# bastienjacquet/CudaDepthMapIntegration

Measured on AMD Instinct MI355X. Metric: Gvoxel-projections/s, higher is better.
Workload: dtype f64

## Files before the change

### cudadepthmapintegration_amd/csrc/dmi_capi_fuse.hip

```cpp
#include "dmi_context.h"

#include <algorithm>
#include <cmath>
#include <cstdlib>
#include <cstring>

using dmi::drain_events;
using dmi::EventPair;
using dmi::fail;
using dmi::flush_zero_fill;
using dmi::FuseArgs;
using dmi::FuseConfig;
using dmi::guarded;
using dmi::MapRec;
using dmi::TileArgs;
using dmi::TileMapRec;

namespace {

int sync_maps(dmi_context *ctx) {
  dmi_context::Views &v = ctx->views;
  const size_t n = v.h_maps.size();
  const size_t cap = std::max<size_t>(64, n * 2);
  bool fresh = false;
// ... 121 lines not shown
  unsigned long long mingled = 0, without = 0, strips = 0, pixels = 0;
  for (const dmi::Batch &bt : v.batches) {
    mingled += bt.mingled_strips;
    without += bt.holes;
    strips += (unsigned long long)bt.n * (unsigned long long)v.W * (unsigned long long)(v.H / 8);
    pixels += (unsigned long long)bt.n * (unsigned long long)v.W * (unsigned long long)v.H;
  }
  return dmi::hole_traits(mingled, without, strips, pixels);
}

int tile_geometry(dmi_context *ctx, const FuseArgs &a, const FuseConfig &cfg, const dmi::TileShape &sh, bool whole_grid, TileArgs *out) {
  TileArgs &t = *out;
  t.nx = a.nx; t.ny = a.ny; t.nz = a.nz; t.W = a.W; t.H = a.H;
  t.first_map = a.first_map; t.n_maps = a.n_maps; t.init_from_grid = a.init_from_grid;
  t.kpad = (a.nz + sh.tk - 1) / sh.tk * sh.tk;
  t.bricks_x = (a.nx + 8 * sh.wx - 1) / (8 * sh.wx);
  t.bricks_y = (a.ny + 8 * sh.wy - 1) / (8 * sh.wy);
  t.bricks_z = t.kpad / sh.tk;
  t.super_x = (t.bricks_x + 3) / 4;
  t.super_y = (t.bricks_y + 3) / 4;
  t.super_z = (t.bricks_z + 1) / 2;
  if (!whole_grid) {
    t.sbz_first = a.k_first / (2 * sh.tk);
    t.super_z = (a.k_first + a.k_count + 2 * sh.tk - 1) / (2 * sh.tk) - t.sbz_first;
  }
  if (t.bricks_x > 2047 || t.bricks_y > 2047 || t.bricks_z > 1023)
    return fail(ctx, DMI_ERR_INVALID_ARGUMENT, "dmi_fuse: more bricks along an axis than the tiled kernel's order entries hold");
  t.slot_base = t.sbz_first * t.super_x * t.super_y * 32;
  t.slot_count = t.super_x * t.super_y * t.super_z * 32;
  const int rc = slot_permutation(ctx, t.super_x, t.super_y, t.super_z, (cfg.variant & dmi::VAR_ZMAJOR_SLOTS) != 0, &t.sb_perm);
  if (rc != DMI_OK) return rc;
  t.xcd_run_wg = 32 * std::max(1, t.super_x * t.super_y);
  if (((int64_t)t.super_x * t.super_y * t.super_z * 32 + 16 * (int64_t)t.xcd_run_wg + 64) > (int64_t)0x7fffffff)
    return fail(ctx, DMI_ERR_INVALID_ARGUMENT, "dmi_fuse: grid too large for one launch");
  t.depth_bytes = (int32_t)((int64_t)a.W * a.H * (ctx->views.depth_f64 ? 8 : 4));
  t.kz0 = a.kz0;
  t.ox = a.ox; t.oy = a.oy; t.oz = a.oz; t.sx = a.sx; t.sy = a.sy; t.sz = a.sz;
  std::memcpy(t.g, a.g, sizeof(t.g));
  t.thick = a.thick; t.delta = a.delta; t.rho_pos = a.rho_pos; t.rho_neg = a.rho_neg;
  t.slope = a.slope; t.free_space = a.free_space;
  t.tile_maps = ctx->views.tile_maps.as<TileMapRec>();
  t.grid = a.grid; t.voxel_hits = a.voxel_hits; t.map_hits = a.map_hits;
  t.rotated = dmi::grid_axis_aligned(ctx->grid) ? 0 : 1;
  t.flags = ((cfg.variant & dmi::VAR_NO_INTERIOR) ? dmi::TILE_FLAG_NO_INTERIOR : 0) |
            ((cfg.variant & dmi::VAR_XCD_RUNS) ? dmi::TILE_FLAG_XCD_RUNS : 0);
  t.maps = ctx->views.maps.as<MapRec>();
  t.wbricks_x = (a.nx + 7) / 8;
  t.wbricks_y = (a.ny + 7) / 8;
  return DMI_OK;
}

int cz_table(dmi_context *ctx, const FuseArgs &a, TileArgs *t) {
  const size_t table_doubles = std::max<size_t>(ctx->views.h_maps.size(), 4) * (size_t)t->kpad;
  const size_t need = table_doubles + (size_t)dmi::kFreeSumsMax + 1;
  const int rc = dmi::ensure_idle_buffer(ctx, ctx->tables.cz_table, need * 8, need * 2 * 8);
  if (rc != DMI_OK) return rc;
  t->cz_table = ctx->tables.cz_table.as<double>();
  if (!a.init_from_grid && !ctx->opt.count_hits && a.n_maps <= dmi::kFreeSumsMax) t->free_sums = t->cz_table + table_doubles;
  return DMI_OK;
}

int zero_row(dmi_context *ctx, TileArgs *t) {
  bool fresh = false;
  const int rc = dmi::ensure_idle_buffer(ctx, ctx->tables.zero_row, (uint64_t)t->class_pitch, (uint64_t)t->class_pitch, &fresh);
  if (rc != DMI_OK) return rc;
  if (fresh) DMI_HIP(ctx, hipMemsetAsync(ctx->tables.zero_row.ptr, dmi::BRICK_MIXED, (size_t)t->class_pitch, ctx->stream));
  t->classes = ctx->tables.zero_row.as<uint8_t>();
  t->class_pitch = 0;
  return DMI_OK;
}

int class_table(dmi_context *ctx, const dmi::TileShape &sh, bool windows, TileArgs *t) {
  const size_t fine_bytes = ((size_t)t->wbricks_x * t->wbricks_y * t->bricks_z * (size_t)t->class_pitch + 255) / 256 * 256;
  const size_t coarse_end = (fine_bytes + (size_t)dmi::coarse_class_bytes(*t, sh.tk) + 255) / 256 * 256;
  const size_t cbytes = coarse_end + (windows ? fine_bytes * sizeof(dmi::WinPair) : 0);
  ctx->tables.coarse_offset = fine_bytes;
  bool fresh = false;
  const int rc = dmi::ensure_idle_buffer(ctx, ctx->tables.classes, cbytes, cbytes, &fresh);
  if (rc != DMI_OK) return rc;
  if (fresh) DMI_HIP(ctx, hipMemsetAsync(ctx->tables.classes.ptr, dmi::BRICK_SKIP, cbytes, ctx->stream));
  t->classes = ctx->tables.classes.as<uint8_t>();
  if (windows) {
    t->win_origin = reinterpret_cast<dmi::WinPair *>(ctx->tables.classes.as<uint8_t>() + coarse_end);
    t->win_delta = (int64_t)reinterpret_cast<intptr_t>(t->win_origin) - 16 * (int64_t)reinterpret_cast<intptr_t>(t->classes);
    t->win_recs = ctx->views.win_recs.as<dmi::WinRec>();
    t->foot_recs = ctx->views.foot_recs.as<dmi::FootRec>();
    t->vb_bytes = (int32_t)std::min<int64_t>(dmi::valid_bits_bytes(ctx->views.W, ctx->views.H), 0x7fffffff);
    t->vb_rowskip = (dmi::valid_bits_tiles_x(ctx->views.W) - 1) * 128;
    t->win_cx = dmi::kValidMargin + ctx->views.W / 2;
    t->win_cy = dmi::kValidMargin + ctx->views.H / 2;
  }
  return DMI_OK;
}

int order_tables(dmi_context *ctx, const dmi::TileShape &sh, int variant, TileArgs *t) {
  const size_t n_slots = (size_t)t->super_x * t->super_y * t->super_z * 32;
  const size_t order_bytes = (n_slots + 1) * sizeof(int32_t), level_bytes = dmi::order_scratch_bytes(n_slots);
  const int rc = dmi::ensure_idle_buffers(ctx, {{&ctx->tables.order, order_bytes, order_bytes}, {&ctx->tables.order_level, level_bytes, level_bytes}});
  if (rc != DMI_OK) return rc;
  t->order = ctx->tables.order.as<int32_t>() + 1;
  t->n_order = ctx->tables.order.as<int32_t>();
  t->order_levels = reinterpret_cast<const int32_t *>(ctx->tables.order_level.as<uint8_t>() + (n_slots + 15) / 16 * 16);
  t->xcd_run_wg = 32 * (4 / (sh.wx * sh.wy));
  if (dmi::cost_order(sh.wx * sh.wy, variant, n_slots)) {
    t->flags |= dmi::TILE_FLAG_COST_ORDER | dmi::TILE_FLAG_XCD_RUNS;
    t->xcd_run_wg = 16;
  }
  return DMI_OK;
}

#ifdef DMI_TUNING
int tuning_hooks(dmi_context *ctx, TileArgs *out) {
  TileArgs &t = *out;
  if (std::getenv("DMI_DEBUG_NO_DEPTH_LOADS")) t.depth_bytes = 0;
  if (std::getenv("DMI_DEBUG_WG_TIMES")) {
    const size_t per_round = 8 * (size_t)t.xcd_run_wg;
    const size_t blocks = ((size_t)t.super_x * t.super_y * t.super_z * 32 + 32 + per_round - 1) / per_round * per_round;
    const size_t bytes = (blocks * 3 + 2) * sizeof(unsigned long long);
    const int rc = dmi::ensure_idle_buffer(ctx, ctx->tables.wg_times, bytes, bytes);
    if (rc != DMI_OK) return rc;
    ctx->tables.wg_times_blocks = blocks;
    DMI_HIP(ctx, hipMemsetAsync(ctx->tables.wg_times.ptr, 0, bytes, ctx->stream));
    t.wg_times = ctx->tables.wg_times.as<unsigned long long>();
    t.wg_times_n = (int64_t)blocks;
  }
  if (const char *e = std::getenv("DMI_DEBUG_PAIRS")) {
    if (!std::strcmp(e, "nowin")) t.flags |= dmi::TILE_FLAG_DBG_SKIP_WINDOW_PAIRS;
    if (!std::strcmp(e, "onlywin")) t.flags |= dmi::TILE_FLAG_DBG_ONLY_WINDOW_PAIRS;
    if (!std::strcmp(e, "nowinloads")) t.flags |= dmi::TILE_FLAG_DBG_NO_WINDOW_LOADS;
  }
  if (const char *e = std::getenv("DMI_XCD_RUN_WG")) {
    t.xcd_run_wg = std::max(1, std::atoi(e));
    if (((int64_t)t.super_x * t.super_y * t.super_z * 32 + 8 * (int64_t)t.xcd_run_wg) > (int64_t)0x7fffffff)
      return fail(ctx, DMI_ERR_INVALID_ARGUMENT, "dmi_fuse: DMI_XCD_RUN_WG makes the launch too large");
  }
  return DMI_OK;
}
#endif

int tile_tables(dmi_context *ctx, const FuseArgs &a, FuseConfig *cfg, const dmi::TileShape &sh, const dmi::HoleTraits &traits, TileArgs *out) {
  TileArgs &t = *out;
  int rc = cz_table(ctx, a, &t);
  if (rc == DMI_OK) rc = dmi::ensure_buffer(ctx, ctx->tables.queue_heads, 128 * sizeof(int32_t));
  if (rc != DMI_OK) return rc;
  t.queue_heads = ctx->tables.queue_heads.as<int32_t>();
  if (dmi::fuse_without_classes(cfg->variant, (int64_t)t.wbricks_x * t.wbricks_y * (int64_t)t.bricks_z, a.n_maps))
    cfg->variant |= dmi::VAR_NO_BRICK_CLASSES;
  t.class_pitch = dmi::class_table_pitch((int32_t)ctx->views.h_maps.size());
  const bool zero_free = dmi::zero_free(a.init_from_grid != 0, ctx->volume.grid_free_of_negative_zero, ctx->opt.count_hits != 0, cfg->variant);
  if (cfg->variant & dmi::VAR_NO_BRICK_CLASSES) {
    rc = zero_row(ctx, &t);
  } else {
    bool any_tier1 = false;
    for (int32_t m = a.first_map; m < a.first_map + a.n_maps && !any_tier1; ++m) any_tier1 = std::isfinite(ctx->views.h_win_recs[(size_t)m].e_abs);
    dmi::WindowsQuestion q;
    q.tier1 = DMI_TIER1 != 0;
    q.general_k = cfg->general_k != 0;
    q.count_hits = cfg->count_hits != 0;
    q.variant = cfg->variant;
    q.holes = cfg->holes != 0;
    q.many_borders = traits.many_borders;
    q.any_tier1 = any_tier1;
    q.zero_free = zero_free;
    q.depth_f64 = ctx->views.depth_f64;
    rc = class_table(ctx, sh, dmi::use_windows(q), &t);
    if (rc == DMI_OK && !(cfg->variant & dmi::VAR_SPATIAL_ORDER)) rc = order_tables(ctx, sh, cfg->variant, &t);
  }
// ... 200 lines not shown
```

### cudadepthmapintegration_amd/csrc/fusion_classify.hip

```cpp
#include <algorithm>
#include <cstring>

#include <stdlib.h>

#include "fusion_kernels.h"
#include "fusion_device.h"

namespace dmi {

namespace {

template <typename T>
__device__ __forceinline__ T cload(const T *p) {
  return *reinterpret_cast<const T __attribute__((address_space(4))) *>(reinterpret_cast<uintptr_t>(p));
}

__device__ __forceinline__ float float_below(double d) {
  float f = (float)d;
  if ((double)f > d) f = nextafterf(f, -__builtin_inff());
  return f;
}
__device__ __forceinline__ float float_above(double d) {
  float f = (float)d;
  if ((double)f < d) f = nextafterf(f, __builtin_inff());
// ... 474 lines not shown
    TileMapRec tr_u;
    if constexpr (views_per_wave == 1) {
      const int mu = __builtin_amdgcn_readfirstlane(m);
      const MapRec *src = maps + mu;
      const TileMapRec *tsrc = a.tile_maps + mu;
#pragma unroll
      for (int q = 8; q < 12; ++q) mr_u.rt[q] = cload(&src->rt[q]);
      mr_u.pyramid = cload(&src->pyramid);
      tr_u.px = cload(&tsrc->px); tr_u.py = cload(&tsrc->py); tr_u.pz = cload(&tsrc->pz); tr_u.p0 = cload(&tsrc->p0);
      tr_u.qx = cload(&tsrc->qx); tr_u.qy = cload(&tsrc->qy); tr_u.qz = cload(&tsrc->qz); tr_u.q0 = cload(&tsrc->q0);
      tr_u.err = cload(&tsrc->err);
      tr_u.cz_err = cload(&tsrc->cz_err);
      tr_u.errz = cload(&tsrc->errz);
      if constexpr (GK) {
        tr_u.sx = cload(&tsrc->sx); tr_u.sy = cload(&tsrc->sy); tr_u.sz = cload(&tsrc->sz); tr_u.s0 = cload(&tsrc->s0);
      }
      mr = &mr_u;
      if (mine) {
        fp = box_footprint<ROT, GK>(a, &mr_u, &tr_u, bx * 8, bx * 8 + 7, by * 8, by * 8 + 7, bz * tk, bz * tk + tk - 1);
      }
    } else {
      if (mine) fp = box_footprint<ROT, GK>(a, mr, a.tile_maps + m, bx * 8, bx * 8 + 7, by * 8, by * 8 + 7, bz * tk, bz * tk + tk - 1);
    }
    const bool query = mine && (fp.query || fp.partial);
    uint8_t cls = fp.cls;
    const int li = query ? query_level<kQueryTiles>(P, max(fp.x1 - fp.x0, fp.y1 - fp.y0) + 1) : 0x7fff;
    bool from_window = false;
    {
      float2 *__restrict__ win_mm = window_mm[wave * views_per_wave + lane / children];
      uint8_t *__restrict__ win_fl = window_fl[wave * views_per_wave + lane / children];
      int li_w = li;
      for (int off = children >> 1; off > 0; off >>= 1) li_w = min(li_w, __shfl_xor(li_w, off, 64));
      if (li_w != 0x7fff) {
        const int L = kPyramidMinLevel + li_w;
        const bool at_level = query && li == li_w;
        int tx0 = at_level ? fp.x0 >> L : 0x7fffffff, ty0 = at_level ? fp.y0 >> L : 0x7fffffff;
        int tx1 = at_level ? fp.x1 >> L : -1, ty1 = at_level ? fp.y1 >> L : -1;
        int wx0 = tx0, wy0 = ty0, wx1 = tx1, wy1 = ty1;
        for (int off = children >> 1; off > 0; off >>= 1) {
          wx0 = min(wx0, __shfl_xor(wx0, off, 64));
          wy0 = min(wy0, __shfl_xor(wy0, off, 64));
          wx1 = max(wx1, __shfl_xor(wx1, off, 64));
          wy1 = max(wy1, __shfl_xor(wy1, off, 64));
        }
        if (wx1 - wx0 < kWindow && wy1 - wy0 < kWindow) {
          const DepthTile *__restrict__ level = mr->pyramid + P.offset[li_w];
          const int pitch = P.width[li_w];
          const int ww = wx1 - wx0 + 1, wh = wy1 - wy0 + 1;
          const int tx = child & 15;
          for (int ty = child >> 4; ty < wh; ty += children / 16)
            if (tx < ww) {
              const DepthTile t = level[(wy0 + ty) * pitch + wx0 + tx];
              win_mm[ty * kWindow + tx] = make_float2(t.dmin, t.dmax);
              win_fl[ty * kWindow + tx] = (uint8_t)t.flags;
            }
          __builtin_amdgcn_fence(__ATOMIC_RELEASE, "wavefront");
          __builtin_amdgcn_wave_barrier();
          __builtin_amdgcn_fence(__ATOMIC_ACQUIRE, "wavefront");
          if (at_level) {
            TileAcc d;
            for (int ty = ty0; ty <= ty1; ++ty)
              for (int tx = tx0; tx <= tx1; ++tx) {
                const int w = (ty - wy0) * kWindow + (tx - wx0);
                const float2 mm = win_mm[w];
                d.add_tile(DepthTile{mm.x, mm.y, (uint32_t)win_fl[w], 0u});
              }
            cls = fp.partial ? border_class<GK>(a, fp, d) : class_from_bounds(a, d, fp.czmin, fp.czmax);
            from_window = true;
          }
          __builtin_amdgcn_fence(__ATOMIC_RELEASE, "wavefront");
          __builtin_amdgcn_wave_barrier();
        }
      }
    }
    if (query && !from_window) {
      const TileAcc d = pyramid_query<kQueryTiles>(mr->pyramid, P, fp.x0, fp.x1, fp.y0, fp.y1);
      cls = fp.partial ? border_class<GK>(a, fp, d) : class_from_bounds(a, d, fp.czmin, fp.czmax);
    }
    if (mine) out[m] = cls;
  }
}

constexpr int kOriginViews = 8;
constexpr uint32_t kNotWanted = 0xfffffffeu;
template <bool ROT>
__global__ __launch_bounds__(256) void window_origin_kernel(const TileArgs a, const MapRec *__restrict__ maps, int tk,
                                                            uint8_t *__restrict__ classes, WinPair *__restrict__ origins,
                                                            int group_views) {
  __shared__ WinPair tile[kOriginViews][256 + 1];
  __shared__ int64_t rows[256];
  const int bz_first = 2 * a.sbz_first;
  const int bz_count = min(2 * a.super_z, a.bricks_z - bz_first);
  const int64_t n_bricks = (int64_t)a.wbricks_x * a.wbricks_y * bz_count;
  const int lane = threadIdx.x & 63;
  const int64_t local = (int64_t)blockIdx.x * 256 + threadIdx.x;
  const bool exists = local < n_bricks;
  const int bx = (int)(local % a.wbricks_x);
  const int64_t t = local / a.wbricks_x;
  const int by = (int)(t % a.wbricks_y), bz = (int)(t / a.wbricks_y) + bz_first;
  const int64_t row = (((int64_t)bz * a.wbricks_y + by) * a.wbricks_x + bx) * a.class_pitch;
  const bool eligible = exists && bz * tk + tk <= a.nz;
  (void)lane;
  double wxa, wya, wza;
  {
    const double gx = a.ox + (bx * 8 + 0.5) * a.sx;
    const double gy = a.oy + (by * 8 + 0.5) * a.sy;
    const double gz = a.oz + ((bz * tk + a.kz0) + 0.5) * a.sz;
    wxa = row4(a.g + 0, gx, gy, gz), wya = row4(a.g + 4, gx, gy, gz), wza = row4(a.g + 8, gx, gy, gz);
  }
  const int m_begin = a.first_map, m_end = a.first_map + a.n_maps;
  const int g_lo = (m_begin & ~3) + blockIdx.y * group_views;
  rows[threadIdx.x] = row;
  uint32_t held[kOriginViews / 4];
#pragma unroll
  for (int g = 0; g < kOriginViews / 4; ++g) {
    const int m4 = g_lo + 4 * g;
    held[g] = (eligible && 4 * g < group_views && m4 < m_end) ? *reinterpret_cast<const uint32_t *>(classes + row + m4) : 0u;
#pragma unroll
    for (int q = 0; q < 4; ++q) tile[4 * g + q][threadIdx.x].origin = kNotWanted;
  }
#pragma unroll
  for (int g = 0; g < kOriginViews / 4; ++g) {
    const int m4 = g_lo + 4 * g;
    if (4 * g >= group_views || m4 >= m_end) break;
    const uint32_t c4 = held[g];
#pragma unroll 1
    for (int q = 0; q < 4; ++q) {
      const int m = m4 + q;
      const uint8_t c = (uint8_t)(c4 >> (8 * q));
      const bool want = eligible && m >= m_begin && m < m_end && (c & 0x1f) == (uint8_t)(BRICK_MIXED | (MIXED_FREE_OR_NODEPTH << 2));
      if (__builtin_amdgcn_ballot_w64(want) == 0) continue;
      WinPair wp;
      wp.origin = kNotWanted;
      wp.ax = wp.ay = wp.acz = 0.f;
      if (cload(&a.win_recs[m].e_abs) < __builtin_inff()) {
        const MapRec *src = maps + m;
        const TileMapRec *tsrc = a.tile_maps + m;
        const FootRec *fr = a.foot_recs + m;
        const float(*scp)[4] = tk == 16 ? fr->s16 : fr->s8;
        if (want) {
          const double cza = ((cload(&src->rt[8]) * wxa + cload(&src->rt[9]) * wya) + cload(&src->rt[10]) * wza) + cload(&src->rt[11]);
          const double hxa = __builtin_fma(cload(&tsrc->cpx), wxa, __builtin_fma(cload(&tsrc->cpy), wya, __builtin_fma(cload(&tsrc->cpz), wza, cload(&tsrc->cp0))));
          const double hya = __builtin_fma(cload(&tsrc->cqx), wxa, __builtin_fma(cload(&tsrc->cqy), wya, __builtin_fma(cload(&tsrc->cqz), wza, cload(&tsrc->cq0))));
          const float hx0 = (float)hxa, hy0 = (float)hya, z0 = (float)cza;
          float umin = __builtin_inff(), umax = -__builtin_inff(), vmin = __builtin_inff(), vmax = -__builtin_inff();
          float zmin = __builtin_inff(), zmax = -__builtin_inff();
#pragma unroll
          for (int cnr = 0; cnr < 8; ++cnr) {
            const float z = z0 + cload(&scp[cnr][2]);
            const float r = __builtin_amdgcn_rcpf(z);
            const float u = (hx0 + cload(&scp[cnr][0])) * r, v = (hy0 + cload(&scp[cnr][1])) * r;
            umin = __builtin_fminf(umin, u), umax = __builtin_fmaxf(umax, u);
            vmin = __builtin_fminf(vmin, v), vmax = __builtin_fmaxf(vmax, v);
            zmin = __builtin_fminf(zmin, z), zmax = __builtin_fmaxf(zmax, z);
          }
          const float umag = __builtin_fmaxf(__builtin_fmaxf(__builtin_fabsf(umin), __builtin_fabsf(umax)), __builtin_fmaxf(__builtin_fabsf(vmin), __builtin_fabsf(vmax)));
          const float e = 2.0f * cload(&fr->ferr) * __builtin_amdgcn_rcpf(zmin) * (1.0f + 0x1p-20f) + (0x1p-19f * umag + 0x1p-12f);
          const bool sane = zmin > 0.0f && zmax <= (float)(kWinCzRatio * (1.0 - 0x1p-20)) * zmin && umin > -65536.0f && umax < 65536.0f &&
                            vmin > -65536.0f && vmax < 65536.0f && e < 0.25f;
          if (sane) {
            const int cxc = a.W / 2, cyc = a.H / 2;
            const int x0 = (int)__builtin_ceilf(umin - 0.5f - e) + cxc, x1 = (int)__builtin_floorf(umax + 0.5f + e) + cxc;
            const int y0 = (int)__builtin_ceilf(vmin - 0.5f - e) + cyc, y1 = (int)__builtin_floorf(vmax + 0.5f + e) + cyc;
            if (x0 >= -kValidMargin && y0 >= -kValidMargin && x1 < a.W + kValidMargin && y1 < a.H + kValidMargin &&
                x1 - x0 < kWindowCols && y1 - y0 < kWindowRows) {
              wp.origin = (uint32_t)(x0 + kValidMargin) | ((uint32_t)(y0 + kValidMargin) << 16);
              wp.ax = (float)(hxa - (double)(x0 + kWinAnchorX - cxc) * cza);
              wp.ay = (float)(hya - (double)(y0 + kWinAnchorY - cyc) * cza);
              wp.acz = z0;
            }
          }
        }
      }
      if (want) {
        if (wp.origin != kNotWanted)
          tile[4 * g + q][threadIdx.x] = wp;
        else
          classes[row + m] = (uint8_t)(c | CLASS_NO_WINDOW);
      }
    }
  }
  __syncthreads();
  const int v = threadIdx.x & (kOriginViews - 1);
  const int m = g_lo + v;
  if (v < group_views && m < m_end) {
#pragma unroll
    for (int it = 0; it < 8; ++it) {
      const int b = (threadIdx.x >> 3) + 32 * it;
      const WinPair wp = tile[v][b];
      if (wp.origin != kNotWanted) origins[rows[b] + m] = wp;
    }
  }
}


__device__ __forceinline__ bool slot_to_brick(const TileArgs &a, int slot, int &bx, int &by, int &bz) {
  const int within = slot & 31;
  const int code = a.sb_perm[(slot - a.slot_base) >> 5];
  const int sbx = code & 1023, sby = (code >> 10) & 1023, sbz = (code >> 20) + a.sbz_first;
  bx = sbx * 4 + (within & 3);
  by = sby * 4 + ((within >> 2) & 3);
  bz = sbz * 2 + (within >> 4);
  return bx < a.bricks_x && by < a.bricks_y && bz < a.bricks_z;
}

constexpr int kWorkLevels = 4;

__global__ __launch_bounds__(256) void brick_work_kernel(const TileArgs a, int wx, int wy, int n_slots,
                                                         uint8_t *__restrict__ level) {
  const int lane = threadIdx.x & 63;
  const int slot = blockIdx.x * 4 + (threadIdx.x >> 6);
  if (slot >= n_slots) return;
  int bx, by, bz;
  if (!slot_to_brick(a, slot + a.slot_base, bx, by, bz)) {
    if (lane == 0) level[slot] = 255;
    return;
  }
  int mixed = 0, total = 0;
  for (int v = 0; v < wy; ++v)
    for (int u = 0; u < wx; ++u) {
      const int wbx = bx * wx + u, wby = by * wy + v;
      if (wbx >= a.wbricks_x || wby >= a.wbricks_y) continue;
      const uint8_t *row = a.classes + (((int64_t)bz * a.wbricks_y + wby) * a.wbricks_x + wbx) * (int64_t)a.class_pitch;
      for (int m = a.first_map + lane; m < a.first_map + a.n_maps; m += 64) mixed += (row[m] & 3) == BRICK_MIXED ? 1 : 0;
      total += a.n_maps;
    }
  for (int off = 32; off > 0; off >>= 1) mixed += __shfl_xor(mixed, off, 64);
  if (lane == 0) level[slot] = mixed * 2 >= total ? 0 : (mixed * 4 >= total ? 1 : (mixed * 16 >= total ? 2 : 3));
}

constexpr int kOrderChunk = 1024;

__global__ __launch_bounds__(kOrderChunk) void order_count_kernel(const uint8_t *__restrict__ level, int n_slots,
                                                                  int *__restrict__ counts) {
  const int s = blockIdx.x * kOrderChunk + threadIdx.x;
  const int l = s < n_slots ? level[s] : 255;
  for (int q = 0; q < kWorkLevels; ++q) {
    const int c = __syncthreads_count(l == q);
    if (threadIdx.x == 0) counts[blockIdx.x * kWorkLevels + q] = c;
  }
}

__global__ __launch_bounds__(1024) void order_base_kernel(int *__restrict__ counts, int n_chunks, int *__restrict__ n_valid) {
  __shared__ int wave_totals[16];
  __shared__ int carry;
  if (threadIdx.x == 0) carry = 0;
  __syncthreads();
  const int lane = threadIdx.x & 63, wave = threadIdx.x >> 6;
  for (int q = 0; q < kWorkLevels; ++q)
    for (int c0 = 0; c0 < n_chunks; c0 += 1024) {
      const int c = c0 + threadIdx.x;
      const int v = c < n_chunks ? counts[c * kWorkLevels + q] : 0;
      int incl = v;
      for (int off = 1; off < 64; off <<= 1) {
        const int up = __shfl_up(incl, off, 64);
        if (lane >= off) incl += up;
      }
      if (lane == 63) wave_totals[wave] = incl;
      __syncthreads();
      int before = carry, all = 0;
      for (int w = 0; w < 16; ++w) {
        if (w < wave) before += wave_totals[w];
        all += wave_totals[w];
      }
      if (c < n_chunks) counts[c * kWorkLevels + q] = before + incl - v;
      __syncthreads();
      if (threadIdx.x == 0) carry += all;
      __syncthreads();
    }
  if (threadIdx.x == 0) *n_valid = carry;
}

__global__ __launch_bounds__(kOrderChunk) void order_scatter_kernel(const TileArgs a, const uint8_t *__restrict__ level,
                                                                    int n_slots, const int *__restrict__ bases,
                                                                    int *__restrict__ order) {
// ... 163 lines not shown
    if (blockIdx.x == 0 && lane == 63) *n_valid = incl;
  }
  __syncthreads();
  const int s = blockIdx.x * kOrderChunk + threadIdx.x;
  const int lv = s < n_slots ? level[s] : 255;
  int pos = -1;
  unsigned long long todo = __builtin_amdgcn_ballot_w64(lv < kCostLevels);
  while (todo) {
    const int leader = __builtin_ctzll(todo);
    const int l0 = __shfl(lv, leader, 64);
    const unsigned long long same = __builtin_amdgcn_ballot_w64(lv == l0) & todo;
    int first = 0;
    if (lane == leader) first = atomicAdd(cursors + l0, __builtin_popcountll(same));
    first = __shfl(first, leader, 64);
    if (lv == l0) pos = base[l0] + first + __builtin_popcountll(same & ((1ull << lane) - 1ull));
    todo &= ~same;
  }
  if (pos >= 0) {
    int bx = 0, by = 0, bz = 0;
    slot_to_brick(a, s + a.slot_base, bx, by, bz);
    order[pos] = pack_brick(bx, by, bz);
  }
}

inline unsigned blocks_of(int64_t n) { return (unsigned)((n + 255) / 256); }

}

PyramidDesc make_pyramid_desc(int W, int H) {
  PyramidDesc P;
  std::memset(&P, 0, sizeof(P));
  int off = 0;
  for (int li = 0; li < kPyramidMaxLevels; ++li) {
    const int L = kPyramidMinLevel + li, S = 1 << L;
    P.width[li] = (W + S - 1) / S;
    P.height[li] = (H + S - 1) / S;
    P.offset[li] = off;
    off += P.width[li] * P.height[li];
    P.n_levels = li + 1;
    if (P.width[li] == 1 && P.height[li] == 1) break;
  }
  P.total_tiles = off;
  return P;
}

hipError_t launch_upload_views(const void *in, int in_is_f64, const double *best_cost, double threshold, void *out, int out_is_f64,
                               int64_t n_maps, int W, int H, const PyramidDesc &P, DepthTile *pyramids, uint8_t *valid, uint32_t *bits,
                               unsigned long long *counters, hipStream_t stream) {
  if (n_maps <= 0) return hipSuccess;
  if (n_maps > 65535) return hipErrorInvalidConfiguration;
  const int cover_x = std::max(W + 2 * kValidMargin, valid_bits_tiles_x(W) * 32);
  const int cover_y = std::max(((H + 2 * kValidMargin + 7) / 8) * 8, valid_bits_tiles_y(H) * 32);
  const dim3 grid((unsigned)((cover_x + 511) / 512), (unsigned)((cover_y + 7) / 8), (unsigned)n_maps);
#define DMI_UPLOAD(IN, OUT)                                                                                                      \
  hipLaunchKernelGGL((upload_views_kernel<IN, OUT>), grid, dim3(512), 0, stream, static_cast<const IN *>(in), best_cost, threshold, \
                     static_cast<OUT *>(out), W, H, P, pyramids, valid, bits, counters)
  if (in_is_f64) {
    if (out_is_f64)
      DMI_UPLOAD(double, double);
    else
      DMI_UPLOAD(double, float);
  } else {
    if (out_is_f64)
      DMI_UPLOAD(float, double);
    else
      DMI_UPLOAD(float, float);
  }
#undef DMI_UPLOAD
  return hipGetLastError();
}

hipError_t launch_build_pyramid_levels(int64_t n_maps, const PyramidDesc &P, DepthTile *pyramids, hipStream_t stream) {
  if (n_maps <= 0 || P.n_levels <= 1) return hipSuccess;
  hipLaunchKernelGGL(pyramid_levels_kernel, dim3((unsigned)n_maps), dim3(1024), 0, stream, P, pyramids);
  return hipGetLastError();
}

hipError_t launch_window_origins(const TileArgs &a, const MapRec *maps_dev, int tk, uint8_t *classes, int general_k,
                                 hipStream_t stream) {
  if (general_k || !a.win_origin || a.n_maps <= 0) return hipSuccess;
  const int bz_count = std::min(2 * a.super_z, a.bricks_z - 2 * a.sbz_first);
  const int64_t n_bricks = (int64_t)a.wbricks_x * a.wbricks_y * bz_count;
  if (n_bricks <= 0) return hipSuccess;
  const int64_t brick_groups = (n_bricks + 255) / 256;
  const int span = a.first_map + a.n_maps - (a.first_map & ~3);
  int group_views = kOriginViews;
  while (group_views > 4 && brick_groups * ((span + group_views - 1) / group_views) < 2048) group_views >>= 1;
  const dim3 grid((unsigned)brick_groups, (unsigned)((span + group_views - 1) / group_views));
  if (a.rotated)
    hipLaunchKernelGGL((window_origin_kernel<true>), grid, dim3(256), 0, stream, a, maps_dev, tk, classes, a.win_origin, group_views);
  else
    hipLaunchKernelGGL((window_origin_kernel<false>), grid, dim3(256), 0, stream, a, maps_dev, tk, classes, a.win_origin, group_views);
  return hipGetLastError();
}

hipError_t launch_classify_bricks(const TileArgs &a, const MapRec *maps_dev, const PyramidDesc &P, int tk, uint8_t *classes,
                                  uint8_t *coarse, int general_k, hipStream_t stream) {
  const int bz_count = std::min(2 * a.super_z, a.bricks_z - 2 * a.sbz_first);
  const int64_t n_bricks = (int64_t)a.wbricks_x * a.wbricks_y * bz_count;
  if (n_bricks <= 0 || a.n_maps <= 0) return hipSuccess;
  if (n_bricks > (int64_t)0x7fffffff || (a.n_maps + 3) / 4 > 65535) return hipErrorInvalidConfiguration;
  const int per_z = 32 / tk;
  const int64_t n_boxes = (int64_t)((a.wbricks_x + 3) / 4) * ((a.wbricks_y + 3) / 4) * ((bz_count + per_z - 1) / per_z);
  const dim3 coarse_grid((unsigned)((n_boxes + 3) / 4), (unsigned)((a.n_maps + 63) / 64));
#define DMI_LAUNCH_COARSE(R, G) \
  hipLaunchKernelGGL((classify_coarse_kernel<R, G>), coarse_grid, dim3(64, 4), 0, stream, a, maps_dev, P, tk, classes, coarse)
  if (a.rotated && general_k)
    DMI_LAUNCH_COARSE(true, true);
  else if (a.rotated)
    DMI_LAUNCH_COARSE(true, false);
  else if (general_k)
    DMI_LAUNCH_COARSE(false, true);
  else
    DMI_LAUNCH_COARSE(false, false);
#undef DMI_LAUNCH_COARSE
  hipError_t e = hipGetLastError();
  if (e != hipSuccess) return e;
  int group_views = 64;
  while (group_views > 8 && n_boxes * ((a.n_maps + group_views - 1) / group_views) < 2048) group_views >>= 1;
  const dim3 fine_grid((unsigned)n_boxes, (unsigned)((a.n_maps + group_views - 1) / group_views));
  [[maybe_unused]] int q = 5;
#ifdef DMI_TUNING
  if (const char *env = getenv("DMI_QUERY_TILES")) q = atoi(env);
#endif
  const bool wide = tk == 8;
#define DMI_LAUNCH_FINE_G(Q, C, R, G) \
  hipLaunchKernelGGL((classify_kernel<Q, C, R, G>), fine_grid, dim3(256), 0, stream, a, maps_dev, P, tk, classes, coarse, group_views)
#define DMI_LAUNCH_FINE_R(Q, C, R)      \
  do {                                  \
    if (general_k)                      \
      DMI_LAUNCH_FINE_G(Q, C, R, true); \
    else                                \
      DMI_LAUNCH_FINE_G(Q, C, R, false);\
  } while (0)
#define DMI_LAUNCH_FINE(Q)                      \
  do {                                          \
    if (wide && a.rotated)                      \
      DMI_LAUNCH_FINE_R(Q, 64, true);           \
    else if (wide)                              \
      DMI_LAUNCH_FINE_R(Q, 64, false);          \
    else if (a.rotated)                         \
      DMI_LAUNCH_FINE_R(Q, 32, true);           \
    else                                        \
      DMI_LAUNCH_FINE_R(Q, 32, false);          \
  } while (0)
#ifdef DMI_TUNING
  if (q <= 2)
    DMI_LAUNCH_FINE(2);
  else if (q == 3)
    DMI_LAUNCH_FINE(3);
  else
#endif
    DMI_LAUNCH_FINE(5);
#undef DMI_LAUNCH_FINE_G
#undef DMI_LAUNCH_FINE_R
#undef DMI_LAUNCH_FINE
  return hipGetLastError();
}

int64_t coarse_class_bytes(const TileArgs &a, int tk) {
  const int per_z = 32 / tk;
  return (int64_t)((a.wbricks_x + 3) / 4) * ((a.wbricks_y + 3) / 4) * ((a.bricks_z + per_z - 1) / per_z) * (int64_t)a.class_pitch;
}

hipError_t launch_order_bricks(const TileArgs &a, int wx, int wy, uint8_t *level, int *order, int *n_valid,
                               hipStream_t stream) {
  const int n_slots = a.super_x * a.super_y * a.super_z * 32;
  if (wx == 1 && wy == 1)
    hipLaunchKernelGGL(brick_work_kernel_1x1, dim3((unsigned)((n_slots + 15) / 16)), dim3(256), 0, stream, a, n_slots, level);
  else
    hipLaunchKernelGGL(brick_work_kernel, dim3((unsigned)((n_slots + 3) / 4)), dim3(256), 0, stream, a, wx, wy, n_slots, level);
// ... 24 lines not shown
```

### cudadepthmapintegration_amd/csrc/fusion_kernels.h

```cpp
#pragma once

#include <hip/hip_runtime.h>
#include <stddef.h>
#include <stdint.h>
#include <string.h>

#include "fusion_launch_rules.h"

struct dmi_context;

namespace dmi {

int grid_pointer_for_sums(::dmi_context *ctx, void **ptr);

struct alignas(16) DepthTile {
  float dmin, dmax;
  uint32_t flags;
  uint32_t pad;
};
enum TileFlags : uint32_t { TILE_HAS_SENTINEL = 1, TILE_HAS_VALID = 2, TILE_HAS_NAN = 4, TILE_PART_HOLE_FREE = 8, TILE_PART_NO_VALID = 16 };
constexpr uint8_t COARSE_CHILDREN_WRITTEN = 0x80;

constexpr int kPyramidMinLevel = 3;
constexpr int kPyramidMaxLevels = 13;
// ... 66 lines not shown
static_assert(sizeof(WinRec) == 64, "WinRec is one cache line");
struct alignas(64) FootRec {
  float s8[8][4];
  float s16[8][4];
  float ferr, pad[15];
};
static_assert(sizeof(FootRec) == 320, "FootRec layout");
#ifdef DMI_WIN_CORNER_ANCHOR
constexpr int kWinAnchorX = 0, kWinAnchorY = 0;
constexpr float kWinC1 = 0.5f - 0x1p-14f;
#else
constexpr int kWinAnchorX = kWindowCols / 2, kWinAnchorY = kWindowRows / 2;
constexpr float kWinC1 = 0.5f - 0x1p-15f;
#endif
constexpr int kWinReach = kWinAnchorY ? kWindowRows - kWinAnchorY : kWindowRows - 1;
constexpr double kWinCzRatio = 1.25;
struct alignas(16) WinPair {
  uint32_t origin;
  float ax, ay, acz;
};
static_assert(sizeof(WinPair) == 16, "WinPair layout");

enum KMode : int {
  K_GENERAL = 0,
  K_PINHOLE_SKEW = 1,
  K_PINHOLE = 2
};

struct FuseArgs {
  int32_t nx, ny, nz;
  int32_t W, H;
  int32_t first_map, n_maps;
  int32_t init_from_grid;
  int32_t kz0, pad1;
  int32_t k_first, k_count;
  double ox, oy, oz;
  double sx, sy, sz;
  double g[12];
  double thick, delta;
  double rho_pos, rho_neg, rho_zero;
  double slope;
  double free_space;
  const MapRec *maps;
  void *grid;
  uint32_t *voxel_hits;
  unsigned long long *map_hits;
};

struct TileArgs {
  int32_t nx, ny, nz, W, H, first_map, n_maps, init_from_grid;
  int32_t kpad;
  int32_t bricks_x, bricks_y, bricks_z;
  int32_t super_x, super_y, super_z;
  int32_t sbz_first, pad3;
  int32_t slot_base, slot_count;
  int32_t depth_bytes;
  int32_t kz0, pad1;
  double ox, oy, oz, sx, sy, sz;
  double g[12];
  double thick, delta, rho_pos, rho_neg, slope, free_space;
  const TileMapRec *tile_maps;
  const double *cz_table;
  void *grid;
  uint32_t *voxel_hits;
  unsigned long long *map_hits;
  const FuseArgs *full;
  const uint8_t *classes;
  int32_t class_pitch;
  int32_t wbricks_x, wbricks_y;
  int32_t xcd_run_wg;
  const int32_t *order;
  const int32_t *n_order;
  unsigned long long behind_mask;
  int32_t rotated;
  int32_t flags;
  const MapRec *maps;
  const int32_t *order_levels;
  const double *free_sums;
  const int32_t *sb_perm;
  unsigned long long *wg_times;
  int64_t wg_times_n;
  int32_t *queue_heads;
  WinPair *win_origin;
  int64_t win_delta;
  const WinRec *win_recs;
  const FootRec *foot_recs;
  int32_t vb_bytes, vb_rowskip;
  int32_t win_cx, win_cy;
};
constexpr int kFreeSumsMax = 4096;
__host__ __device__ inline int32_t pack_brick(int bx, int by, int bz) { return (int32_t)((uint32_t)bx | ((uint32_t)by << 11) | ((uint32_t)bz << 22)); }
static_assert(offsetof(TileArgs, nx) == 0 && offsetof(TileArgs, nz) == 8 && offsetof(TileArgs, kpad) == 32 &&
                  offsetof(TileArgs, bricks_x) == 36 && offsetof(TileArgs, bricks_z) == 44 && offsetof(TileArgs, sbz_first) == 60,
              "TileArgs head layout");
enum TileKernelFlags : int32_t {
  TILE_FLAG_NO_INTERIOR = 1,
  TILE_FLAG_XCD_RUNS = 2,
  TILE_FLAG_COST_ORDER = 4,
  TILE_FLAG_DBG_SKIP_WINDOW_PAIRS = 256,
  TILE_FLAG_DBG_ONLY_WINDOW_PAIRS = 512,
  TILE_FLAG_DBG_NO_WINDOW_LOADS = 1024
};

enum BrickClass : uint8_t {
  BRICK_MIXED = 0,
  BRICK_FREE = 1,
  BRICK_BEHIND = 2,
  BRICK_SKIP = 3
};

enum MixedReason : uint8_t {
  MIXED_UNSPECIFIED = 0,
  MIXED_DEGENERATE = 1,
  MIXED_CAMERA_PLANE = 2,
  MIXED_IMAGE_BORDER = 3,
  MIXED_NAN_DEPTH = 4,
  MIXED_SENTINEL_AND_DEPTH = 5,
  MIXED_NEAR_SURFACE = 6,
  MIXED_FREE_OR_NODEPTH = 7
};

struct FuseConfig {
  int depth_is_f64;
  int grid_is_f64;
  int k_mode;
  int count_hits;
  int variant;
  int use_tile;
  int general_k;
  int holes;
};


constexpr int kMaxColumnHeight = 16;
struct TileShape {
  int tk, wx, wy;
};
TileShape tile_shape(int variant, bool depth_is_f64, bool rotated, bool general_k);

hipError_t launch_fuse(const FuseArgs &args, const FuseConfig &cfg, hipStream_t stream);

hipError_t launch_fuse_tiled(const TileArgs &args, const MapRec *maps_dev, const FuseConfig &cfg, const PyramidDesc &pyramid,
                             uint8_t *order_scratch, uint8_t *coarse_classes, hipEvent_t before_main_kernel,
                             hipStream_t stream);

hipError_t launch_widen_depth(const float *in, double *out, int64_t n, hipStream_t stream);
hipError_t launch_convert_grid(const void *in, int in_is_f64, void *out, int64_t n, hipStream_t stream);

hipError_t launch_fp64_probe(double *out, int blocks, int iters, hipStream_t stream);

PyramidDesc make_pyramid_desc(int W, int H);
hipError_t launch_upload_views(const void *in, int in_is_f64, const double *best_cost, double threshold, void *out, int out_is_f64,
                               int64_t n_maps, int W, int H, const PyramidDesc &desc, DepthTile *pyramids, uint8_t *valid, uint32_t *bits,
                               unsigned long long *counters, hipStream_t stream);
hipError_t launch_build_pyramid_levels(int64_t n_maps, const PyramidDesc &desc, DepthTile *pyramids, hipStream_t stream);
hipError_t launch_window_origins(const TileArgs &args, const MapRec *maps_dev, int tk, uint8_t *classes, int general_k,
                                 hipStream_t stream);
hipError_t launch_classify_bricks(const TileArgs &args, const MapRec *maps_dev, const PyramidDesc &desc, int tk,
                                  uint8_t *classes, uint8_t *coarse, int general_k, hipStream_t stream);
int64_t coarse_class_bytes(const TileArgs &args, int tk);
size_t order_scratch_bytes(size_t n_slots);
hipError_t launch_order_bricks(const TileArgs &args, int wx, int wy, uint8_t *level, int *order, int *n_valid,
                               hipStream_t stream);

hipError_t launch_cell_to_point(const void *cells, int cells_are_f64, double *points, int nx, int ny, int nz,
                                hipStream_t stream);

// ... 128 lines not shown
```

### cudadepthmapintegration_amd/csrc/fusion_launch_rules.h

```cpp
#pragma once
#include <stddef.h>
#include <stdint.h>

namespace dmi {

constexpr int64_t kNoClassesMaxBricks = 1024;
constexpr int kNoClassesMaxViews = 48;

enum VariantBits : int {
  VAR_EXACT_DIVISION = 1,
  VAR_GENERAL_K = 2,
  VAR_BLOCK_SHAPE_MASK = 12,
  VAR_FORCE_GENERAL = 16,
  VAR_TILE_SHAPE_MASK = 0xE0,
  VAR_TILE_SHAPE_SHIFT = 5,
  VAR_NO_BRICK_CLASSES = 256,
  VAR_SPATIAL_ORDER = 512,
  VAR_FIXED_TILE_SHAPE = 4096,
  VAR_KEEP_BEHIND_ADDS = 1024,
  VAR_NO_INTERIOR = 2048,
  VAR_XCD_RUNS = 8192,
  VAR_ZMAJOR_SLOTS = 16384,
  VAR_PERSISTENT_ALWAYS = 32768,
  VAR_PERSISTENT_NEVER = 65536,
  VAR_BRICK_CLASSES_ALWAYS = 131072,
  VAR_NO_WINDOWS = 262144,
  VAR_WINDOWS_ALWAYS = 524288,
  VAR_COST_ORDER = 1048576,
  VAR_NO_COST_ORDER = 2097152
};

constexpr int kCostOrderMaxSlots = 0;

struct HoleTraits {
  bool scattered = false;
  bool holes = false;
  bool tall_by_holes = false;
  bool many_borders = false;
  bool mostly_empty = false;
};

inline HoleTraits hole_traits(unsigned long long mingled, unsigned long long without, unsigned long long strips, unsigned long long pixels) {
  HoleTraits h;
  h.scattered = without <= 6 * mingled;
  h.holes = h.scattered && mingled * 160 > strips;
  h.tall_by_holes = h.scattered && mingled * 80 > strips;
  h.many_borders = mingled * 25 > strips;
  h.tall_by_holes = h.tall_by_holes || h.many_borders;
  if (!h.holes) h.mostly_empty = without * 4 >= pixels && pixels > 0;
  return h;
}

inline int with_default_tile_shape(int variant, bool tiled, const HoleTraits &h, int32_t nx, int32_t ny, int32_t nz) {
  if (tiled && !(variant & (VAR_TILE_SHAPE_MASK | VAR_FIXED_TILE_SHAPE))) {
    const int64_t bricks16 = (int64_t)((nx + 15) / 16) * ((ny + 15) / 16) * ((nz + 15) / 16);
    if (bricks16 <= 32768 && !(h.tall_by_holes && bricks16 >= 4096) && !(h.mostly_empty && bricks16 >= 13824))
      variant |= 7 << VAR_TILE_SHAPE_SHIFT;
  }
  return variant;
}

inline bool fuse_without_classes(int variant, int64_t wave_bricks, int32_t views) {
  if (variant & VAR_NO_BRICK_CLASSES) return true;
  return !(variant & VAR_BRICK_CLASSES_ALWAYS) && wave_bricks <= kNoClassesMaxBricks && views < kNoClassesMaxViews;
}

inline int32_t class_table_pitch(int32_t resident_views) {
  int32_t pitch = 64;
  while (pitch < resident_views) pitch *= 2;
  return pitch;
}

inline bool zero_free(bool init_from_grid, bool grid_free_of_negative_zero, bool count_hits, int variant) {
  return (!init_from_grid || grid_free_of_negative_zero) && !count_hits && !(variant & VAR_KEEP_BEHIND_ADDS);
}

struct WindowsQuestion {
  bool tier1;
  bool general_k;
  bool count_hits;
  int variant;
  bool holes, many_borders;
  bool any_tier1;
  bool zero_free;
  bool depth_f64;
};
inline bool use_windows(const WindowsQuestion &q) {
  return q.tier1 && !q.general_k && !q.count_hits && !(q.variant & (VAR_NO_WINDOWS | VAR_NO_INTERIOR)) &&
         (q.holes || q.many_borders || (q.variant & VAR_WINDOWS_ALWAYS)) && q.any_tier1 && q.zero_free && !q.depth_f64;
}

inline bool cost_order(int waves_per_workgroup, int variant, size_t n_slots) {
  return waves_per_workgroup == 1 && !(variant & VAR_NO_COST_ORDER) && ((variant & VAR_COST_ORDER) || n_slots <= (size_t)kCostOrderMaxSlots);
}

}
```

### cudadepthmapintegration_amd/csrc/fusion_tile.hip

```cpp
#include <stdlib.h>

#include <algorithm>
#include <type_traits>

#include "fusion_kernels.h"
#include "fusion_device.h"

#ifndef DMI_T1_CHAINS
#define DMI_T1_CHAINS 4
#endif
#ifndef DMI_T1_COLUMN_CHAINS
#define DMI_T1_COLUMN_CHAINS 2
#endif
#if !defined(DMI_TUNING) && (defined(DMI_EXP_SKIP_WINDOW_VIEWS) || defined(DMI_EXP_SAME_REC) || defined(DMI_EXP_NO_WINDOW_LOADS) || \
                             defined(DMI_EXP_NO_LANE_MARGIN))
#error "a DMI_EXP_* switch that changes results was defined without DMI_TUNING"
#endif

namespace dmi {

int tile_shape_index(int variant);

namespace {

// ... 325 lines not shown
  if (p_order) {
    bx = entry & 2047, by = (entry >> 11) & 2047, bz = (int)((unsigned)entry >> 22);
  } else {
    const int within = p & 31;
    const int code = cload(kb->sb_perm + (p >> 5));
    const int sbx = code & 1023, sby = (code >> 10) & 1023, sbz = (code >> 20) + head1[7];
    bx = sbx * 4 + (within & 3), by = sby * 4 + ((within >> 2) & 3), bz = sbz * 2 + (within >> 4);
  }
  if ((bx >= head1[1]) | (by >= head1[2]) | (bz >= head1[3])) DMI_NEXT_BRICK

#ifdef DMI_TUNING
  unsigned long long wg_t0 = 0;
  if (kb->wg_times) wg_t0 = __builtin_amdgcn_s_memrealtime();
  unsigned dbg_cols = 0, dbg_redo = 0;
  unsigned dbg_win = 0, dbg_win_early = 0;
  unsigned dbg_win_redo = 0;
#endif
  const int wbx = bx * WX + (w % WX), wby = by * WY + (w / WX);
  if ((wbx >= kb->wbricks_x) | (wby >= kb->wbricks_y)) DMI_NEXT_BRICK
  const int i = wbx * kLX + (lane % kLX);
  const int j = wby * kLY + (lane / kLX);
  const int k0 = bz * TK;
  const int kcount = head0[2] - k0 < TK ? head0[2] - k0 : TK;
  const bool lane_ok = (i < head0[0]) & (j < head0[1]);

  const kernarg_t kg = kb;
  const double gx = kg->ox + (i + 0.5) * kg->sx;
  const double gy = kg->oy + (j + 0.5) * kg->sy;
  const double gz0 = kg->oz + ((k0 + kg->kz0) + 0.5) * kg->sz;
  double gm[12];
#pragma unroll
  for (int q = 0; q < 12; ++q) gm[q] = kg->g[q];
  const double wx = ROT ? gm[0] * gx + gm[1] * gy : row4(gm + 0, gx, gy, gz0);
  const double wy = ROT ? gm[4] * gx + gm[5] * gy : row4(gm + 4, gx, gy, gz0);
  const double wz0 = ROT ? gm[8] * gx + gm[9] * gy : row4(gm + 8, gx, gy, gz0);


  uint32_t nh[COUNT ? TK : 1];
#ifndef DMI_EXP_INIT_ALWAYS_OLD
  if constexpr (!PERSIST) {
    if (kg->init_from_grid) {
      GridT held[TK];
      const int ic = i < head0[0] ? i : head0[0] - 1, jc = j < head0[1] ? j : head0[1] - 1;
      const GridT *column = static_cast<const GridT *>(kg->grid) + ((int64_t)k0 * kg->ny + jc) * kg->nx + ic;
      const int64_t plane_in = (int64_t)kg->ny * kg->nx;
#pragma unroll
      for (int kk = 0; kk < TK; ++kk) held[kk] = column[(int64_t)(kk < kcount ? kk : kcount - 1) * plane_in];
#pragma unroll
      for (int kk = 0; kk < TK; ++kk) acc_set<BASE, TK>(kk, (double)held[kk]);
    } else {
#pragma unroll
      for (int kk = 0; kk < TK; ++kk) acc_set<BASE, TK>(kk, 0.0);
    }
  } else
#endif
  {
#pragma unroll
    for (int kk = 0; kk < TK; ++kk) {
      double v0 = 0.0;
      if (kg->init_from_grid && lane_ok && kk < kcount)
        v0 = (double)static_cast<const GridT *>(kg->grid)[(((int64_t)(k0 + kk)) * kg->ny + j) * kg->nx + i];
      acc_set<BASE, TK>(kk, v0);
    }
  }
  if (COUNT) {
#pragma unroll
    for (int kk = 0; kk < TK; ++kk) nh[kk] = 0;
  }

  const mask_t m_lane_ok_brick = ballot(lane_ok);

  const unsigned long long *crow = reinterpret_cast<const unsigned long long *>(
      KA(classes) + (((int64_t)bz * KA(wbricks_y) + wby) * KA(wbricks_x) + wbx) * (int64_t)KA(class_pitch));

  int n_uniform = (!COUNT && KA(free_sums) != nullptr) ? 0 : -1;
  unsigned long long cnext = cload(crow + (first_map >> 3));
  [[maybe_unused]] uint32_t pair_a = 0, pair_b = 0;
  for (int wbase = first_map & ~7; wbase < m_end; wbase += 8) {
    if constexpr (WIN) {
      if ((wbase & 24) == 0 || wbase == (first_map & ~7)) {
        const kernarg_t ko = KFRESH();
        if (ko->win_origin) {
          typedef uint32_t u32x2 __attribute__((ext_vector_type(2)));
          const u32x2 *row = reinterpret_cast<const u32x2 *>(ko->win_delta + 16 * (int64_t)reinterpret_cast<intptr_t>(crow));
          const u32x2 pr = row[2 * (wbase & ~31) + lane];
          pair_a = pr.x;
          pair_b = pr.y;
        }
      }
    }
    const unsigned long long cword = cnext | ((cnext >> 1) & (ZF ? 0x0101010101010101ull : KC(behind_mask)));
    if (wbase + 8 < m_end) cnext = cload(crow + (wbase >> 3) + 1);
    const unsigned long long nonskip = cword ^ 0x0303030303030303ull;
    unsigned long long todo = (nonskip | (nonskip >> 1)) & 0x0101010101010101ull;
    if (wbase < first_map) todo &= ~0ull << ((first_map - wbase) * 8);
    if (wbase + 8 > m_end) todo &= (1ull << ((m_end - wbase) * 8)) - 1;
    unsigned long long fr = COUNT ? 0ull : (todo & cword & ~(cword >> 1));
    unsigned long long other = todo ^ fr;
  for (;;) {
    const unsigned long long below = (other - 1) & ~other;
    const int n_free_now = __builtin_popcountll(fr & below);
    fr &= ~below;
    if (n_uniform >= 0) {
      n_uniform += n_free_now;
    } else {
      for (int n_free = n_free_now; n_free > 0; --n_free) {
#pragma unroll
        for (int q = 0; q < TK; q += 8) acc_add8_all<BASE, TK>(q, free_space);
      }
    }
    if (other == 0) break;
    const int vbit = __builtin_ctzll(other);
    other &= other - 1;
    const int m = wbase + (vbit >> 3);
    if (n_uniform >= 0) {
      const double v = cload(KC(free_sums) + n_uniform);
#pragma unroll
      for (int q = 0; q < TK; ++q) acc_set<BASE, TK>(q, v);
      n_uniform = -1;
    }
    const unsigned cbyte = (unsigned)(cword >> vbit) & 0x3fu;
    const unsigned cls = cbyte & 3u;
    if (cls != BRICK_MIXED) {
      const double v = cls == BRICK_FREE ? free_space : 0.0;
#pragma unroll
      for (int q = 0; q < TK; q += 8) acc_add8_all<BASE, TK>(q, v);
      if (COUNT) {
#pragma unroll
        for (int q = 0; q < TK; ++q) nh[q] += lane_ok ? 1u : 0u;
        const uint32_t hits = (uint32_t)__popcll(m_lane_ok_brick) * (uint32_t)kcount;
        if (hits != 0 && lane == 0) atomicAdd(&KC(map_hits)[m], (unsigned long long)hits);
      }
      continue;
    }
    [[maybe_unused]] const bool has_window = WIN && cbyte == ((unsigned)MIXED_FREE_OR_NODEPTH << 2 | BRICK_MIXED) && kcount == TK;
#ifdef DMI_TUNING
    ++dbg_cols;
    if ((kflags & TILE_FLAG_DBG_SKIP_WINDOW_PAIRS) && has_window) continue;
    if ((kflags & TILE_FLAG_DBG_ONLY_WINDOW_PAIRS) && !has_window) continue;
#endif
    if constexpr (WIN) {
      if (has_window) {
#ifdef DMI_TUNING
        ++dbg_win;
        if (dbg_cols == dbg_win) ++dbg_win_early;
#endif
        const int pl = (m & 31) * 2;
        const uint32_t org = (uint32_t)__builtin_amdgcn_readlane((int)pair_a, pl);
        const unsigned long long A2 = (unsigned long long)(uint32_t)__builtin_amdgcn_readlane((int)pair_b, pl) |
                                      ((unsigned long long)(uint32_t)__builtin_amdgcn_readlane((int)pair_a, pl + 1) << 32);
        const float acz = __int_as_float(__builtin_amdgcn_readlane((int)pair_b, pl + 1));
        const int x0p = (int)(org & 0xffffu), y0p = (int)(org >> 16);
        const kernarg_t kw = KFRESH();
        typedef uint32_t u32x16 __attribute__((ext_vector_type(16)));
        const WinRec *const wrec = kw->win_recs + m;
        const u32x16 R = *reinterpret_cast<const u32x16 __attribute__((address_space(4))) *>(reinterpret_cast<uintptr_t>(wrec));
#ifndef DMI_NO_WINREC_PREFETCH
        int next_rec;
        asm volatile("s_load_dword %0, %1, 0x40" : "=&s"(next_rec) : "s"(wrec), "s"(R[15]));
#endif
        const __amdgpu_buffer_rsrc_t brsrc = __builtin_amdgcn_make_buffer_rsrc(
            reinterpret_cast<uint32_t *>((uintptr_t)R[0] | ((uintptr_t)R[1] << 32)), (short)0, kw->vb_bytes, 0x00020000);
        const unsigned lin = ((unsigned)lane << 2) + ((unsigned)y0p << 2);
        const unsigned off = __umul24(lin >> 7, (unsigned)kw->vb_rowskip) + lin + (((unsigned)x0p >> 5) << 7);
#ifdef DMI_TUNING
        uint32_t w_lo, w_hi;
        if (kflags & TILE_FLAG_DBG_NO_WINDOW_LOADS) {
          w_lo = off * 0x9e3779b9u, w_hi = ~w_lo;
// ... 886 lines not shown
```

Baseline: 3050.

## Store window-origin pairs in view-block-major layout instead of brick-major

Changes the WinPair origin table layout from brick-major with the class pitch to blocks of 32 views, indexed by brick within each view block. The origin kernel now handles 64 bricks per workgroup across four wave sets covering 32 views, and writes the pairs out contiguously through a shared-memory transpose. The tile kernel computes the new index from the brick offset and view block. The aim is denser, coalesced writes in the origin kernel and smaller strides in the tile kernel's reads, at the cost of extra index arithmetic and a narrower brick dimension per workgroup.

```diff
diff --git a/cudadepthmapintegration_amd/csrc/dmi_capi_fuse.hip b/cudadepthmapintegration_amd/csrc/dmi_capi_fuse.hip
--- a/cudadepthmapintegration_amd/csrc/dmi_capi_fuse.hip
+++ b/cudadepthmapintegration_amd/csrc/dmi_capi_fuse.hip
@@ -227,7 +227,7 @@
   t->classes = ctx->tables.classes.as<uint8_t>();
   if (windows) {
     t->win_origin = reinterpret_cast<dmi::WinPair *>(ctx->tables.classes.as<uint8_t>() + coarse_end);
-    t->win_delta = (int64_t)reinterpret_cast<intptr_t>(t->win_origin) - 16 * (int64_t)reinterpret_cast<intptr_t>(t->classes);
+    t->n_class_bricks = (int64_t)t->wbricks_x * t->wbricks_y * t->bricks_z;
     t->win_recs = ctx->views.win_recs.as<dmi::WinRec>();
     t->foot_recs = ctx->views.foot_recs.as<dmi::FootRec>();
     t->vb_bytes = (int32_t)std::min<int64_t>(dmi::valid_bits_bytes(ctx->views.W, ctx->views.H), 0x7fffffff);
diff --git a/cudadepthmapintegration_amd/csrc/fusion_classify.hip b/cudadepthmapintegration_amd/csrc/fusion_classify.hip
--- a/cudadepthmapintegration_amd/csrc/fusion_classify.hip
+++ b/cudadepthmapintegration_amd/csrc/fusion_classify.hip
@@ -580,18 +580,28 @@
 }
 
 constexpr int kOriginViews = 8;
+#ifdef DMI_WINPAIR_BRICK_MAJOR
+constexpr int kOriginBricks = 256, kOriginWaveSets = 1, kOriginAlign = 4;
+#else
+constexpr int kOriginBricks = 64, kOriginWaveSets = 4, kOriginAlign = kWinPairBlockViews;
+static_assert(kOriginViews * kOriginWaveSets == kWinPairBlockViews, "a workgroup's views are one block of the pair table");
+#endif
 constexpr uint32_t kNotWanted = 0xfffffffeu;
 template <bool ROT>
 __global__ __launch_bounds__(256) void window_origin_kernel(const TileArgs a, const MapRec *__restrict__ maps, int tk,
                                                             uint8_t *__restrict__ classes, WinPair *__restrict__ origins,
                                                             int group_views) {
-  __shared__ WinPair tile[kOriginViews][256 + 1];
+  __shared__ WinPair tile[kOriginViews * kOriginWaveSets][kOriginBricks + 1];
+#ifdef DMI_WINPAIR_BRICK_MAJOR
   __shared__ int64_t rows[256];
+#endif
   const int bz_first = 2 * a.sbz_first;
   const int bz_count = min(2 * a.super_z, a.bricks_z - bz_first);
   const int64_t n_bricks = (int64_t)a.wbricks_x * a.wbricks_y * bz_count;
   const int lane = threadIdx.x & 63;
-  const int64_t local = (int64_t)blockIdx.x * 256 + threadIdx.x;
+  const int tb = threadIdx.x % kOriginBricks;
+  const int wset = kOriginWaveSets > 1 ? __builtin_amdgcn_readfirstlane(threadIdx.x / kOriginBricks) : 0;
+  const int64_t local = (int64_t)blockIdx.x * kOriginBricks + tb;
   const bool exists = local < n_bricks;
   const int bx = (int)(local % a.wbricks_x);
   const int64_t t = local / a.wbricks_x;
@@ -607,15 +617,21 @@
     wxa = row4(a.g + 0, gx, gy, gz), wya = row4(a.g + 4, gx, gy, gz), wza = row4(a.g + 8, gx, gy, gz);
   }
   const int m_begin = a.first_map, m_end = a.first_map + a.n_maps;
-  const int g_lo = (m_begin & ~3) + blockIdx.y * group_views;
+  const int g_wg = (m_begin & ~(kOriginAlign - 1)) + blockIdx.y * (group_views * kOriginWaveSets);
+  const int slot0 = wset * group_views;
+  const int g_lo = g_wg + slot0;
+#ifdef DMI_WINPAIR_BRICK_MAJOR
   rows[threadIdx.x] = row;
+#endif
   uint32_t held[kOriginViews / 4];
 #pragma unroll
   for (int g = 0; g < kOriginViews / 4; ++g) {
     const int m4 = g_lo + 4 * g;
     held[g] = (eligible && 4 * g < group_views && m4 < m_end) ? *reinterpret_cast<const uint32_t *>(classes + row + m4) : 0u;
-#pragma unroll
-    for (int q = 0; q < 4; ++q) tile[4 * g + q][threadIdx.x].origin = kNotWanted;
+    if (4 * g < group_views) {
+#pragma unroll
+      for (int q = 0; q < 4; ++q) tile[slot0 + 4 * g + q][tb].origin = kNotWanted;
+    }
   }
 #pragma unroll
   for (int g = 0; g < kOriginViews / 4; ++g) {
@@ -672,13 +688,14 @@
       }
       if (want) {
         if (wp.origin != kNotWanted)
-          tile[4 * g + q][threadIdx.x] = wp;
+          tile[slot0 + 4 * g + q][tb] = wp;
         else
           classes[row + m] = (uint8_t)(c | CLASS_NO_WINDOW);
       }
     }
   }
   __syncthreads();
+#ifdef DMI_WINPAIR_BRICK_MAJOR
   const int v = threadIdx.x & (kOriginViews - 1);
   const int m = g_lo + v;
   if (v < group_views && m < m_end) {
@@ -689,6 +706,18 @@
       if (wp.origin != kNotWanted) origins[rows[b] + m] = wp;
     }
   }
+#else
+  const int wg_views = group_views * kOriginWaveSets;
+  const int lg = 31 - __builtin_clz((unsigned)wg_views);
+  const int64_t brick0 = (int64_t)blockIdx.x * kOriginBricks + (int64_t)bz_first * a.wbricks_y * a.wbricks_x;
+  for (int e = threadIdx.x; e < kOriginBricks * wg_views; e += 256) {
+    const int b = e >> lg, v = e & (wg_views - 1);
+    const int m = g_wg + v;
+    if (m >= m_end) continue;
+    const WinPair wp = tile[v][b];
+    if (wp.origin != kNotWanted) origins[win_pair_index(brick0 + b, m, a.n_class_bricks)] = wp;
+  }
+#endif
 }
 
 
@@ -1018,11 +1047,13 @@
   const int bz_count = std::min(2 * a.super_z, a.bricks_z - 2 * a.sbz_first);
   const int64_t n_bricks = (int64_t)a.wbricks_x * a.wbricks_y * bz_count;
   if (n_bricks <= 0) return hipSuccess;
-  const int64_t brick_groups = (n_bricks + 255) / 256;
-  const int span = a.first_map + a.n_maps - (a.first_map & ~3);
+  const int64_t brick_groups = (n_bricks + kOriginBricks - 1) / kOriginBricks;
+  const int span = a.first_map + a.n_maps - (a.first_map & ~(kOriginAlign - 1));
   int group_views = kOriginViews;
-  while (group_views > 4 && brick_groups * ((span + group_views - 1) / group_views) < 2048) group_views >>= 1;
-  const dim3 grid((unsigned)brick_groups, (unsigned)((span + group_views - 1) / group_views));
+  const auto view_groups = [&](int gv) { return (span + gv * kOriginWaveSets - 1) / (gv * kOriginWaveSets); };
+  while (group_views > 4 && brick_groups * view_groups(group_views) < 2048) group_views >>= 1;
+  if (brick_groups > (int64_t)0x7fffffff || a.n_class_bricks > (int64_t)0x7fffffff) return hipErrorInvalidConfiguration;
+  const dim3 grid((unsigned)brick_groups, (unsigned)view_groups(group_views));
   if (a.rotated)
     hipLaunchKernelGGL((window_origin_kernel<true>), grid, dim3(256), 0, stream, a, maps_dev, tk, classes, a.win_origin, group_views);
   else
diff --git a/cudadepthmapintegration_amd/csrc/fusion_kernels.h b/cudadepthmapintegration_amd/csrc/fusion_kernels.h
--- a/cudadepthmapintegration_amd/csrc/fusion_kernels.h
+++ b/cudadepthmapintegration_amd/csrc/fusion_kernels.h
@@ -172,7 +172,7 @@
   int64_t wg_times_n;
   int32_t *queue_heads;
   WinPair *win_origin;
-  int64_t win_delta;
+  int64_t n_class_bricks;
   const WinRec *win_recs;
   const FootRec *foot_recs;
   int32_t vb_bytes, vb_rowskip;
diff --git a/cudadepthmapintegration_amd/csrc/fusion_launch_rules.h b/cudadepthmapintegration_amd/csrc/fusion_launch_rules.h
--- a/cudadepthmapintegration_amd/csrc/fusion_launch_rules.h
+++ b/cudadepthmapintegration_amd/csrc/fusion_launch_rules.h
@@ -71,6 +71,16 @@
   return pitch;
 }
 
+#if defined(__HIP__)
+#define DMI_RULES_HD __host__ __device__
+#else
+#define DMI_RULES_HD
+#endif
+constexpr int kWinPairBlockViews = 32;
+DMI_RULES_HD inline int64_t win_pair_index(int64_t brick, int32_t view, int64_t n_class_bricks) {
+  return (((int64_t)(view >> 5) * n_class_bricks + brick) << 5) + (view & 31);
+}
+
 inline bool zero_free(bool init_from_grid, bool grid_free_of_negative_zero, bool count_hits, int variant) {
   return (!init_from_grid || grid_free_of_negative_zero) && !count_hits && !(variant & VAR_KEEP_BEHIND_ADDS);
 }
diff --git a/cudadepthmapintegration_amd/csrc/fusion_tile.hip b/cudadepthmapintegration_amd/csrc/fusion_tile.hip
--- a/cudadepthmapintegration_amd/csrc/fusion_tile.hip
+++ b/cudadepthmapintegration_amd/csrc/fusion_tile.hip
@@ -431,8 +431,15 @@
         const kernarg_t ko = KFRESH();
         if (ko->win_origin) {
           typedef uint32_t u32x2 __attribute__((ext_vector_type(2)));
-          const u32x2 *row = reinterpret_cast<const u32x2 *>(ko->win_delta + 16 * (int64_t)reinterpret_cast<intptr_t>(crow));
-          const u32x2 pr = row[2 * (wbase & ~31) + lane];
+          const uint64_t row_off = (uint64_t)(reinterpret_cast<intptr_t>(crow) - reinterpret_cast<intptr_t>(ko->classes));
+#ifdef DMI_WINPAIR_BRICK_MAJOR
+          const u32x2 *row = reinterpret_cast<const u32x2 *>(reinterpret_cast<intptr_t>(ko->win_origin) + 16 * (int64_t)row_off) + 2 * (wbase & ~31);
+#else
+          const uint64_t brick = row_off >> __builtin_ctz((unsigned)ko->class_pitch);
+          const uint64_t block_first = (uint64_t)(uint32_t)ko->n_class_bricks * (uint32_t)(wbase >> 5);
+          const u32x2 *row = reinterpret_cast<const u32x2 *>(ko->win_origin + ((block_first + brick) << 5));
+#endif
+          const u32x2 pr = row[lane];
           pair_a = pr.x;
           pair_b = pr.y;
         }
```

Result: faster. 3097, median of 6 (+1.5%).
